# openMVG/openMVG

Measured on AMD Instinct MI355X. Metric: descriptor pairs/s (brute-force L2 2-NN + ratio matching), higher is better.
Workload: dtype i8 (int32 accumulate); 1 GPU; 1000 images x 2000 SIFT-like uint8x128 descriptors, exhaustive pairs (499500 image pairs, 499500 on rank 0), ratio 0.8; parallelism=pair-sharded x1, no collective

## Files before the change

### openmvg_amd/csrc/mvgx_bruteforce.hip

```cpp
#include <hip/hip_runtime.h>

#include <algorithm>
#include <cmath>
#include <cstring>
#include <deque>
#include <mutex>
#include <random>
#include <thread>
#include <vector>

#include "mvgx_buffers.h"
#include "mvgx_common.h"
#include "mvgx_match_batch.h"

namespace {

using mvgx::DevBuf;
using mvgx::PinnedBuf;
using mvgx::set_error;

constexpr int kQBlock = 256;
constexpr uint32_t kRowBits = 22;

struct HamParams {
// ... 546 lines not shown
      norms[r] = nn;
    }
    if ((rc = c->d_norms.ensure(norms.size()))) return rc;
    MVGX_HIP(hipMemcpyAsync(c->d_norms.p, norms.data(), norms.size() * sizeof(uint32_t), hipMemcpyHostToDevice, c->stream));
  }
  if (n_images)
    MVGX_HIP(hipMemcpyAsync(c->d_n.p, c->h_n.data(), n_images * sizeof(uint32_t), hipMemcpyHostToDevice, c->stream));
  MVGX_HIP(hipStreamSynchronize(c->stream));
  return MVGX_OK;
}

int bf_run(BfCtx* c, const uint32_t* pairs_IJ, uint64_t n_pairs, float ratio, mvgx_match_stats* stats) {
  MVGX_REQUIRE(c && (pairs_IJ || n_pairs == 0), MVGX_ERR_ARG, "run: NULL argument");
  MVGX_REQUIRE(c->nw != 0 || c->n_images == 0, MVGX_ERR_STATE, "run before set_regions");
  int rc;
  if (c->kind != 3 && (rc = check_ratio(ratio, "ratio"))) return rc;
  MVGX_HIP(hipSetDevice(c->device));
  if ((rc = check_pairs_in_range(pairs_IJ, n_pairs, c->n_images, "run"))) return rc;
  c->res_offsets.assign(n_pairs + 1, 0);
  c->res_ij.clear();
  mvgx_match_stats st;
  memset(&st, 0, sizeof(st));
  st.variant = (c->kind == 0 ? 100 : c->kind == 1 ? 200 : c->kind == 2 ? 300 : 400) + c->nw;
  float kernel_ms = 0.f;
  MVGX_HIP(hipEventRecord(c->ev0, c->stream));
  const uint64_t B = batch_size(c->batch_pairs, c->qstride);
  MVGX_REQUIRE(B * std::max<uint32_t>(c->qstride, 1) < (1ull << 32), MVGX_ERR_UNSUPPORTED,
               "images of %u descriptor slots: a 16-pair batch overflows the 32-bit match offsets of the device path", c->qstride);
  for (uint64_t p0 = 0; p0 < n_pairs; p0 += B) {
    const uint32_t nb = (uint32_t)std::min<uint64_t>(B, n_pairs - p0);
    const uint32_t blocks_per_pair = std::max<uint32_t>(1, c->qstride / kQBlock);
    if ((rc = c->hp_pairs.ensure(nb)) || (rc = c->hp_work.ensure((size_t)nb * blocks_per_pair))) return rc;
    uint32_t n_work = 0;
    for (uint32_t k = 0; k < nb; ++k) {
      const uint32_t I = pairs_IJ[2 * (p0 + k)], J = pairs_IJ[2 * (p0 + k) + 1];
      c->hp_pairs.p[k] = make_uint2(I, J);
      const uint32_t nI = c->h_n[I], nJ = c->h_n[J];
      if (c->kind == 3 ? (nI == 0 || nJ == 0) : (nI < 2 || nJ == 0)) continue;
      for (uint32_t q0 = 0; q0 < nJ; q0 += kQBlock) c->hp_work.p[n_work++] = make_uint2(k, q0);
      st.n_pairs += 1;
      st.n_desc_pairs += (uint64_t)nI * nJ;
    }
    if ((rc = c->d_pairs.ensure(nb)) || (rc = c->d_work.ensure(std::max<uint32_t>(n_work, 1))) ||
        (rc = c->d_best.ensure((size_t)nb * std::max<uint32_t>(c->qstride, 1))) || (rc = c->d_count.ensure(nb)) ||
        (rc = c->d_offsets.ensure((size_t)nb + 1)) || (rc = c->hp_offsets.ensure((size_t)nb + 1)))
      return rc;
    MVGX_HIP(hipMemcpyAsync(c->d_pairs.p, c->hp_pairs.p, nb * sizeof(uint2), hipMemcpyHostToDevice, c->stream));
    if (n_work) MVGX_HIP(hipMemcpyAsync(c->d_work.p, c->hp_work.p, n_work * sizeof(uint2), hipMemcpyHostToDevice, c->stream));
    MVGX_HIP(hipMemsetAsync(c->d_count.p, 0, nb * sizeof(uint32_t), c->stream));
    if (n_work) {
      MVGX_HIP(hipEventRecord(c->evk0, c->stream));
      if (c->kind == 3) {
        CasParams cp;
        cp.words = c->d_words.p; cp.hash = reinterpret_cast<const uint32_t*>(c->d_hash.p); cp.bids = c->d_bids.p; cp.bstart = c->d_bstart.p; cp.items = c->d_items.p;
        cp.img_row_off = c->d_row_off.p; cp.img_n = c->d_n.p; cp.pairs = c->d_pairs.p; cp.work = c->d_work.p; cp.best = c->d_best.p;
        cp.count = c->d_count.p; cp.qstride = c->qstride; cp.n_groups = c->cas_groups; cp.n_buckets = c->cas_buckets; cp.ratio_sq = ratio;
        if (c->cas_float) hipLaunchKernelGGL((cascade_match_kernel<64, 2, true>), dim3(n_work), dim3(kQBlock), 0, c->stream, cp);
        else if (c->nw == 36) hipLaunchKernelGGL((cascade_match_kernel<36, 5, false>), dim3(n_work), dim3(kQBlock), 0, c->stream, cp);
        else hipLaunchKernelGGL((cascade_match_kernel<32, 4, false>), dim3(n_work), dim3(kQBlock), 0, c->stream, cp);
      } else if (c->kind == 0) {
        HamParams hp;
        hp.words = c->d_words.p; hp.img_row_off = c->d_row_off.p; hp.img_n = c->d_n.p; hp.pairs = c->d_pairs.p; hp.work = c->d_work.p;
        hp.best = c->d_best.p; hp.count = c->d_count.p; hp.qstride = c->qstride; hp.ratio = ratio;
        if (c->nw == 8) hipLaunchKernelGGL(hamming_top2_ratio_kernel<8>, dim3(n_work), dim3(kQBlock), 0, c->stream, hp);
        else hipLaunchKernelGGL(hamming_top2_ratio_kernel<16>, dim3(n_work), dim3(kQBlock), 0, c->stream, hp);
      } else if (c->kind == 2) {
        L2uParams up;
        up.words = c->d_words.p; up.norms = c->d_norms.p; up.img_row_off = c->d_row_off.p; up.img_n = c->d_n.p; up.pairs = c->d_pairs.p;
        up.work = c->d_work.p; up.best = c->d_best.p; up.count = c->d_count.p; up.qstride = c->qstride; up.ratio_sq = ratio;
        if (c->nw == 16) hipLaunchKernelGGL(l2u8_top2_ratio_kernel<16>, dim3(n_work), dim3(kQBlock), 0, c->stream, up);
        else if (c->nw == 32) hipLaunchKernelGGL(l2u8_top2_ratio_kernel<32>, dim3(n_work), dim3(kQBlock), 0, c->stream, up);
        else hipLaunchKernelGGL(l2u8_top2_ratio_kernel<36>, dim3(n_work), dim3(kQBlock), 0, c->stream, up);
      } else {
        L2fParams fp;
        fp.rows = reinterpret_cast<const float*>(c->d_words.p); fp.img_row_off = c->d_row_off.p; fp.img_n = c->d_n.p;
        fp.pairs = c->d_pairs.p; fp.work = c->d_work.p; fp.best = c->d_best.p; fp.count = c->d_count.p; fp.qstride = c->qstride;
        fp.ratio_sq = ratio;
        hipLaunchKernelGGL(l2f_top2_ratio_kernel<64>, dim3(n_work), dim3(kQBlock), 0, c->stream, fp);
      }
      MVGX_HIP(hipGetLastError());
      MVGX_HIP(hipEventRecord(c->evk1, c->stream));
      st.n_kernel_launches += 1;
    }
    hipLaunchKernelGGL(scan_counts_kernel, dim3(1), dim3(1024), 0, c->stream, c->d_count.p, nb, c->d_offsets.p);
    MVGX_HIP(hipGetLastError());
    MVGX_HIP(hipMemcpyAsync(c->hp_offsets.p, c->d_offsets.p, ((size_t)nb + 1) * sizeof(uint32_t), hipMemcpyDeviceToHost, c->stream));
    MVGX_HIP(hipStreamSynchronize(c->stream));
    if (n_work) {
      float ms = 0.f;
      MVGX_HIP(hipEventElapsedTime(&ms, c->evk0, c->evk1));
      kernel_ms += ms;
    }
    const uint32_t total = c->hp_offsets.p[nb];
    const uint64_t base = c->res_offsets[p0];
    for (uint32_t k = 0; k <= nb; ++k) c->res_offsets[p0 + k] = base + c->hp_offsets.p[k];
    st.n_matches += total;
    if (total) {
      if ((rc = c->d_ij.ensure(total))) return rc;
      hipLaunchKernelGGL(compact_matches_kernel, dim3((nb + 3) / 4), dim3(256), 0, c->stream, c->d_best.p, c->d_offsets.p, c->d_pairs.p,
                         c->d_n.p, c->d_row_off.p, (const uint32_t*)nullptr, nb, c->qstride, c->d_ij.p);
      MVGX_HIP(hipGetLastError());
      const size_t old = c->res_ij.size();
      c->res_ij.resize(old + (size_t)total * 2);
      MVGX_HIP(hipMemcpyAsync(c->res_ij.data() + old, c->d_ij.p, (size_t)total * sizeof(uint2), hipMemcpyDeviceToHost, c->stream));
      MVGX_HIP(hipStreamSynchronize(c->stream));
    }
  }
  MVGX_HIP(hipEventRecord(c->ev1, c->stream));
  MVGX_HIP(hipEventSynchronize(c->ev1));
  float ms = 0.f;
  MVGX_HIP(hipEventElapsedTime(&ms, c->ev0, c->ev1));
  st.total_ms = ms;
  st.kernel_ms = kernel_ms;
  if (stats) *stats = st;
  return MVGX_OK;
}

template <typename Ctx>
int bf_create_as(int kind, int device, Ctx** out) {
  MVGX_REQUIRE(out, MVGX_ERR_ARG, "create: NULL out");
  *out = nullptr;
  Ctx* c = new Ctx();
  const int rc = bf_create(kind, device, c);
  if (rc) { delete c; return rc; }
  *out = c;
  return MVGX_OK;
}

}

extern "C" {

int mvgx_hamming_create(int device, mvgx_hamming_ctx** out) { return bf_create_as(0, device, out); }
int mvgx_hamming_destroy(mvgx_hamming_ctx* c) { delete c; return MVGX_OK; }
int mvgx_hamming_set_option(mvgx_hamming_ctx* c, const char* key, int64_t value) { return bf_set_option(c, key, value); }

int mvgx_hamming_set_regions(mvgx_hamming_ctx* c, const uint8_t* const* desc_rows, const uint32_t* n_desc, uint32_t n_images,
                             uint32_t desc_bytes) {
  MVGX_REQUIRE(c && (n_images == 0 || (desc_rows && n_desc)), MVGX_ERR_ARG, "mvgx_hamming_set_regions: NULL argument");
  MVGX_REQUIRE(desc_bytes >= 1 && desc_bytes <= 64, MVGX_ERR_UNSUPPORTED,
               "binary descriptor of %u bytes unsupported (device path: 1..64 bytes; AKAZE MLDB is 64)", desc_bytes);
  return bf_set_regions(c, desc_rows, n_desc, n_images, desc_bytes, desc_bytes <= 32 ? 8 : 16);
}

int mvgx_hamming_run(mvgx_hamming_ctx* c, const uint32_t* pairs_IJ, uint64_t n_pairs, float dist_ratio, mvgx_match_stats* stats) {
  return bf_run(c, pairs_IJ, n_pairs, dist_ratio, stats);
}

int mvgx_hamming_results(mvgx_hamming_ctx* c, const uint64_t** offsets, const uint32_t** ij) {
  MVGX_REQUIRE(c && offsets && ij, MVGX_ERR_ARG, "mvgx_hamming_results: NULL argument");
  *offsets = c->res_offsets.data();
  *ij = c->res_ij.data();
  return MVGX_OK;
}

int mvgx_l2f_create(int device, mvgx_l2f_ctx** out) { return bf_create_as(1, device, out); }
int mvgx_l2f_destroy(mvgx_l2f_ctx* c) { delete c; return MVGX_OK; }
int mvgx_l2f_set_option(mvgx_l2f_ctx* c, const char* key, int64_t value) { return bf_set_option(c, key, value); }

int mvgx_l2f_set_regions(mvgx_l2f_ctx* c, const float* const* desc_rows, const uint32_t* n_desc, uint32_t n_images, uint32_t dim) {
  MVGX_REQUIRE(c && (n_images == 0 || (desc_rows && n_desc)), MVGX_ERR_ARG, "mvgx_l2f_set_regions: NULL argument");
  MVGX_REQUIRE(dim == 64, MVGX_ERR_UNSUPPORTED,
               "float descriptors of length %u unsupported (device path: 64 = AKAZE_Float_Regions)", dim);
  return bf_set_regions(c, reinterpret_cast<const uint8_t* const*>(desc_rows), n_desc, n_images, dim * 4, dim);
}

int mvgx_l2f_run(mvgx_l2f_ctx* c, const uint32_t* pairs_IJ, uint64_t n_pairs, float ratio_sq, mvgx_match_stats* stats) {
// ... 243 lines not shown
```

### openmvg_amd/csrc/mvgx_match.hip

```cpp
#include <hip/hip_runtime.h>

#include <algorithm>
#include <atomic>
#include <climits>
#include <condition_variable>
#include <cstdint>
#include <cstdlib>
#include <cstring>
#include <functional>
#include <mutex>
#include <string>
#include <thread>
#include <vector>

#include "mvgx_buffers.h"
#include "mvgx_common.h"
#include "mvgx_match_batch.h"

namespace {

using mvgx::DevBuf;
using mvgx::PinnedBuf;
using mvgx::set_error;

// ... 895 lines not shown
    const int8_t* qsrc = p.tiles + (size_t)(tileJ0 + qt0) * kTileBytes + lane_chunk;
#pragma unroll
    for (int n = 0; n < kNBh; ++n)
#pragma unroll
      for (int ks = 0; ks < 2; ++ks) b[n][ks] = *reinterpret_cast<const v4i*>(qsrc + (n >> 1) * kTileBytes + (n & 1) * 256 + ks * 2048);
  }
  const int8_t* gI = p.tiles + (size_t)tileI0 * kTileBytes;
  const int* gC = p.cinit + (size_t)tileI0 * kTileRows;

  uint32_t qperm[kNBh];
  int qn[kNBh];
#pragma unroll
  for (int n = 0; n < kNBh; ++n) {
    const bool inb = lane < 16 && qt0 + (uint32_t)(n >> 1) < ntJpad;
    const size_t qs = (size_t)tileJ0 * kTileRows + (qt0 + (uint32_t)(n >> 1)) * kTileRows + (uint32_t)(n & 1) * 16 + (uint32_t)(lane & 15);
    qperm[n] = inb ? p.perm[qs] : kNoMatch;
    qn[n] = inb ? p.qnorm[qs] : 0;
  }

  int TP[kNBh][4], TW[kNBh][4], Q1[kNBh], Q2[kNBh], Qg[kNBh];
#pragma unroll
  for (int n = 0; n < kNBh; ++n) {
#pragma unroll
    for (int c = 0; c < 4; ++c) { TP[n][c] = kNegInit; TW[n][c] = kNegInit; }
    Q1[n] = kNegInit; Q2[n] = kNegInit; Qg[n] = 0;
  }

  stage_half_glds_asm(smem, gI, gC, wave, lane);
#pragma unroll
  for (int n = 0; n < kNBh; ++n) {
#pragma unroll
    for (int ks = 0; ks < 2; ++ks) asm volatile("" : "+v"(b[n][ks]));
    asm volatile("" : "+v"(qperm[n]), "+v"(qn[n]));
  }

  for (int hw = 0; hw < nhalf; ++hw) {
    asm volatile("s_waitcnt vmcnt(0)" ::: "memory");
    __syncthreads();
    char* buf = smem + (hw & 1) * kHalfStageBytes;
    char* nbuf = smem + ((hw + 1) & 1) * kHalfStageBytes;
    if (hw + 1 < nhalf)
      stage_half_glds_asm(nbuf, gI + (size_t)(hw + 1) * kHalfTiles * kTileBytes, gC + (hw + 1) * kHalfTiles * kTileRows, wave, lane);

    const int nt = min(kHalfTiles, ntI - hw * kHalfTiles);
    const char* wb = buf + lane_chunk;
    const char* wc = buf + kHalfTiles * kTileBytes + g4 * 16;
    v4i accA[4], accB[4];
#pragma unroll
    for (int i = 0; i < 4; ++i) accB[i] = v4i{kNegInit, kNegInit, kNegInit, kNegInit};
    v4i a0[2], a1[2], c0, c1;
    a0[0] = *reinterpret_cast<const v4i*>(wb);
    a0[1] = *reinterpret_cast<const v4i*>(wb + 2048);
    c0 = *reinterpret_cast<const v4i*>(wc);
    for (int t = 0; t < nt; ++t) {
      const int tn = min(t + 1, nt - 1);
      MVGX_GROUP16(accA, 0, a0, c0)
      a1[0] = *reinterpret_cast<const v4i*>(wb + t * kTileBytes + 256);
      a1[1] = *reinterpret_cast<const v4i*>(wb + t * kTileBytes + 256 + 2048);
      c1 = *reinterpret_cast<const v4i*>(wc + t * (kTileRows * 4) + 64);
      MVGX_EPI16(accB, 0, 1)
      MVGX_MIX16(3)
      MVGX_GROUP16(accB, 0, a1, c1)
      a0[0] = *reinterpret_cast<const v4i*>(wb + tn * kTileBytes);
      a0[1] = *reinterpret_cast<const v4i*>(wb + tn * kTileBytes + 2048);
      c0 = *reinterpret_cast<const v4i*>(wc + tn * (kTileRows * 4));
      MVGX_EPI16(accA, 0, 0)
      MVGX_MIX16(3)
    }
    MVGX_EPI16(accB, 0, 1)
    if ((hw & 1) || hw + 1 == nhalf) {
#pragma unroll
      for (int n = 0; n < kNBh; ++n) fold_window<4>(TW[n], TP[n], Q1[n], Q2[n], Qg[n], hw >> 1);
    }
  }

#pragma unroll
  for (int n = 0; n < kNBh; ++n) MVGX_FINISH16(n, qt0 + (uint32_t)(n >> 1) < ntJpad, qperm[n] != kNoMatch)
}
#undef MVGX_FINISH16
#undef MVGX_GROUP16
#undef MVGX_EPI16
#undef MVGX_MIX16

__device__ __forceinline__ int sum8_dpp(int v) {
  v += __builtin_amdgcn_update_dpp(0, v, 0xB1, 0xF, 0xF, true);
  v += __builtin_amdgcn_update_dpp(0, v, 0x4E, 0xF, 0xF, true);
  v += __builtin_amdgcn_update_dpp(0, v, 0x141, 0xF, 0xF, true);
  return v;
}
__device__ __forceinline__ int min16_dpp(int v) {
  v = min(v, __builtin_amdgcn_update_dpp(INT_MAX, v, 0xB1, 0xF, 0xF, false));
  v = min(v, __builtin_amdgcn_update_dpp(INT_MAX, v, 0x4E, 0xF, 0xF, false));
  v = min(v, __builtin_amdgcn_update_dpp(INT_MAX, v, 0x141, 0xF, 0xF, false));
  v = min(v, __builtin_amdgcn_update_dpp(INT_MAX, v, 0x140, 0xF, 0xF, false));
  return v;
}

template <bool kWaveUnits>
__global__ __launch_bounds__(256) void l2_verify_kernel(MatchParams p) {
  const int lane = threadIdx.x & 63;
  const int wave = threadIdx.x >> 6;
  uint32_t pair, qt0, I, tileI0, tileJ0, qend;
  const uint8_t* rowsJ = nullptr;
  if constexpr (kWaveUnits) {
    const uint4* rec = p.work8 + (size_t)kRecQuads * blockIdx.x;
    const uint4 wun = rec[1 + __builtin_amdgcn_readfirstlane(wave)];
    pair = wun.x; tileJ0 = wun.y; qt0 = wun.z; qend = wun.w;
    tileI0 = rec[0].x;
    const uint2 ij = p.pairs[pair];
    I = ij.x;
    rowsJ = p.rows_u8 + p.img_row_off[ij.y] * kDim;
  } else {
    const uint2 wk = p.work[blockIdx.x];
    const uint2 ij = p.pairs[wk.x];
    pair = wk.x; qt0 = wk.y + (uint32_t)wave * kNQ;
    I = ij.x;
    tileI0 = p.img_tile_off[I]; tileJ0 = p.img_tile_off[ij.y];
    qend = (p.img_tile_off[ij.y + 1] - tileJ0) * kTileRows;
  }
  const uint32_t nEvenI = p.img_neven[I], nOddI = p.img_n[I] - nEvenI;
  const int l16 = lane & 15, sub = lane >> 4;
  uint32_t accepted = 0;
  for (int part = 0; part < 2; ++part) {
    const uint32_t q0 = qt0 * kTileRows + (uint32_t)part * 64;
    const uint32_t q = q0 + lane;
    const bool inb = q < qend;
    const uint32_t code = inb ? p.best[(size_t)pair * p.qstride + q] : kNoMatch;
    unsigned long long todo = __ballot(code != kNoMatch);
    while (todo) {
      unsigned long long m = todo;
      for (int i = 0; i < sub; ++i) m &= m - 1;
      const bool active = m != 0;
      const int src = active ? __builtin_ctzll(m) : 0;
      for (int i = 0; i < 4; ++i) todo &= todo - 1;
      const uint32_t cc = (uint32_t)__shfl((int)code, src);
      const uint32_t qs = q0 + (uint32_t)src;
      const int s1 = cc & 7, hw = (cc >> 3) & 1, g1 = (int)(cc >> 4);
      const int piece = l16 & 7, rsel = l16 >> 3;
      const int mrow = slot_row(2 * s1 + rsel, hw);
      const size_t slot0 = (size_t)tileI0 * kTileRows + (active ? (size_t)g1 * kWinTiles * kTileRows + mrow : 0);
      const size_t slotQ = (size_t)tileJ0 * kTileRows + (active ? qs : 0);
      const size_t o = (size_t)pair * p.qstride + (active ? qs : 0);
      const uint32_t tt = (uint32_t)g1 * kWinTiles + (uint32_t)piece;
      const size_t slotI = active ? slot0 + (size_t)piece * kTileRows : slot0;
      const bool valid = active && (tt * 16u + (uint32_t)(2 * s1 + rsel)) < (hw ? nOddI : nEvenI);
      int4 va[8];
#pragma unroll
      for (int c = 0; c < 8; ++c)
        va[c] = *reinterpret_cast<const int4*>(p.rows_slot + (slot0 + (active ? (size_t)c * kTileRows : 0)) * kDim + piece * 16);
      int4 vb;
      if constexpr (kWaveUnits) {
        vb = *reinterpret_cast<const int4*>(rowsJ + (size_t)(active ? qs : 0) * kDim + piece * 16);
        vb.x ^= (int)0x80808080u; vb.y ^= (int)0x80808080u; vb.z ^= (int)0x80808080u; vb.w ^= (int)0x80808080u;
      } else {
        vb = *reinterpret_cast<const int4*>(p.rows_slot + slotQ * kDim + piece * 16);
      }
      const int2 f = p.cd[o];
      const int f_d0 = f.x, f_d1 = f.y;
      int nb = __builtin_amdgcn_sdot4(vb.x, vb.x, 0, false);
      nb = __builtin_amdgcn_sdot4(vb.y, vb.y, nb, false);
      nb = __builtin_amdgcn_sdot4(vb.z, vb.z, nb, false);
      nb = __builtin_amdgcn_sdot4(vb.w, vb.w, nb, false);
      nb = sum8_dpp(nb);
      int dot = 0, na = 0;
#pragma unroll
      for (int c = 0; c < 8; ++c) {
        int part = __builtin_amdgcn_sdot4(va[c].x, vb.x, 0, false);
        part = __builtin_amdgcn_sdot4(va[c].y, vb.y, part, false);
        part = __builtin_amdgcn_sdot4(va[c].z, vb.z, part, false);
        part = __builtin_amdgcn_sdot4(va[c].w, vb.w, part, false);
        part = sum8_dpp(part);
        dot = (c == piece) ? part : dot;
        int sq = __builtin_amdgcn_sdot4(va[c].x, va[c].x, 0, false);
        sq = __builtin_amdgcn_sdot4(va[c].y, va[c].y, sq, false);
        sq = __builtin_amdgcn_sdot4(va[c].z, va[c].z, sq, false);
        sq = __builtin_amdgcn_sdot4(va[c].w, va[c].w, sq, false);
        sq = sum8_dpp(sq);
        na = (c == piece) ? sq : na;
      }
      const int d = valid ? na + nb - 2 * dot : INT_MAX;
      const int key = min16_dpp(valid ? ((d << 4) | l16) : INT_MAX);
      const int wl = key & 15, dbest = key >> 4;
      const int second = min16_dpp((l16 == wl) ? INT_MAX : d);
      bool ok = false;
      if (active && l16 == wl) {
        if (key == INT_MAX || dbest != f_d0) atomicAdd(p.errflag, 1u);
        const int d1 = min(f_d1, second);
        ok = __int2float_rn(dbest) < __fmul_rn(p.ratio_sq, __int2float_rn(d1));
        p.best[o] = ok ? p.perm[slotI] : kNoMatch;
      }
      accepted += (uint32_t)__popcll(__ballot(ok));
    }
  }
  if (lane == 0 && accepted) atomicAdd(&p.count[pair], accepted);
}

__global__ __launch_bounds__(256) void count_candidates_kernel(const uint32_t* __restrict__ best, size_t n,
                                                               uint32_t* __restrict__ counter) {
  __shared__ uint32_t s_sum;
  if (threadIdx.x == 0) s_sum = 0;
  __syncthreads();
  uint32_t c = 0;
  const size_t base = (size_t)blockIdx.x * 16384;
  for (int k = 0; k < 64; ++k) {
    const size_t i = base + (size_t)k * 256 + threadIdx.x;
    if (i < n && best[i] != kNoMatch) ++c;
  }
  const unsigned long long m = __ballot(c != 0);
  (void)m;
  for (int off = 32; off > 0; off >>= 1) c += __shfl_down(c, off);
  if ((threadIdx.x & 63) == 0 && c) atomicAdd(&s_sum, c);
  __syncthreads();
  if (threadIdx.x == 0 && s_sum) atomicAdd(counter, s_sum);
}

__global__ __launch_bounds__(256) void count_candidates_units_kernel(MatchParams p, uint32_t* __restrict__ counter) {
  __shared__ uint32_t s_sum;
  if (threadIdx.x == 0) s_sum = 0;
  __syncthreads();
  const int lane = threadIdx.x & 63, wave = threadIdx.x >> 6;
  const uint4 wun = p.work8[(size_t)kRecQuads * blockIdx.x + 1 + wave];
  uint32_t c = 0;
  for (int part = 0; part < 2; ++part) {
    const uint32_t q = wun.z * kTileRows + (uint32_t)part * 64 + (uint32_t)lane;
    const bool cand = q < wun.w && p.best[(size_t)wun.x * p.qstride + q] != kNoMatch;
    c += (uint32_t)__popcll(__ballot(cand));
  }
  if (lane == 0 && c) atomicAdd(&s_sum, c);
  __syncthreads();
  if (threadIdx.x == 0 && s_sum) atomicAdd(counter, s_sum);
}

__global__ __launch_bounds__(256) void l2_top2_ratio_naive_kernel(MatchParams p) {
  const uint2 wk = p.work[blockIdx.x];
  const uint2 ij = p.pairs[wk.x];
  const uint32_t I = ij.x, J = ij.y;
  const uint32_t nI = p.img_n[I], nJ = p.img_n[J];
  const uint8_t* rowsI = p.rows_u8 + p.img_row_off[I] * kDim;
  const uint8_t* rowsJ = p.rows_u8 + p.img_row_off[J] * kDim;
  for (uint32_t q = wk.y * kTileRows + threadIdx.x; q < min(nJ, (wk.y + kBlockQTiles) * kTileRows);
       q += blockDim.x) {
    uint32_t qv[32];
#pragma unroll
    for (int k = 0; k < 32; ++k) qv[k] = reinterpret_cast<const uint32_t*>(rowsJ + (size_t)q * kDim)[k];
    int d0 = INT_MAX, d1 = INT_MAX;
    uint32_t i0 = 0;
    for (uint32_t i = 0; i < nI; ++i) {
      const uint32_t* dbr = reinterpret_cast<const uint32_t*>(rowsI + (size_t)i * kDim);
      int d = 0;
#pragma unroll
      for (int k = 0; k < 32; ++k) {
        const uint32_t x = qv[k], y = dbr[k];
#pragma unroll
        for (int bb = 0; bb < 4; ++bb) {
          const int df = (int)((x >> (8 * bb)) & 0xFF) - (int)((y >> (8 * bb)) & 0xFF);
          d += df * df;
        }
      }
      if (d < d0) { d1 = d0; d0 = d; i0 = i; }
      else if (d < d1) { d1 = d; }
    }
    const bool ok = __int2float_rn(d0) < __fmul_rn(p.ratio_sq, __int2float_rn(d1));
    p.best[(size_t)wk.x * p.qstride + p.rowpos[p.img_row_off[J] + q]] = ok ? i0 : kNoMatch;
    if (ok) atomicAdd(&p.count[wk.x], 1u);
  }
}


}

struct mvgx_match_ctx {
  int device = 0;
// ... 110 lines not shown
      out[2 * n] = make_uint4(k, qt, c->h_tile_off[I], c->h_tile_off[J]);
      out[2 * n + 1] = make_uint4(c->h_ntiles[I], c->h_tile_off[J + 1] - c->h_tile_off[J], 0, 0);
      ++n;
    }
  }
  return n;
}
uint32_t build_records(const mvgx_match_ctx* c, const uint32_t* ij, uint32_t nb, uint4* out) {
  uint32_t n_rec = 0, rec_used = kWaves, rec_I = 0;
  for (uint32_t k = 0; k < nb; ++k) {
    const uint32_t I = ij[2 * k], J = ij[2 * k + 1];
    if (!pair_has_work(c, I, J)) continue;
    const uint32_t ntJq = c->h_qtile_off[J + 1] - c->h_qtile_off[J];
    for (uint32_t qt = 0; qt < ntJq; qt += kNQ) {
      if (rec_used == kWaves || rec_I != I) {
        uint4* r = out + (size_t)kRecQuads * n_rec++;
        r[0] = make_uint4(c->h_tile_off[I], c->h_ntiles[I], 0, 0);
        for (int w = 0; w < kWaves; ++w) r[1 + w] = make_uint4(0, c->h_qtile_off[I], 0, 0);
        rec_used = 0; rec_I = I;
      }
      out[(size_t)kRecQuads * (n_rec - 1) + 1 + rec_used++] = make_uint4(k, c->h_qtile_off[J], qt, c->h_n[J]);
    }
  }
  return n_rec;
}

template <typename T>
int upload_list(DevBuf<T>& d, const PinnedBuf<T>& h, size_t n, hipStream_t stream) {
  const int rc = d.ensure(std::max<size_t>(n, 1));
  if (rc) return rc;
  if (n) MVGX_HIP(hipMemcpyAsync(d.p, h.p, n * sizeof(T), hipMemcpyHostToDevice, stream));
  return MVGX_OK;
}

int prep_regions(mvgx_match_ctx* c) {
  const uint32_t n_images = c->n_images;
  c->h_tile_off.assign(n_images + 1, 0);
  c->h_row_off.assign(n_images + 1, 0);
  c->h_ntiles.assign(n_images + 1, 0);
  c->h_qtile_off.assign(n_images + 1, 0);
  uint32_t max_n = 0;
  for (uint32_t k = 0; k < n_images; ++k) {
    c->h_row_off[k + 1] = c->h_row_off[k] + c->h_n[k];
    c->h_qtile_off[k + 1] = c->h_qtile_off[k] + (c->h_n[k] + kTileRows - 1) / kTileRows;
    max_n = std::max(max_n, c->h_n[k]);
  }
  const uint64_t total_rows = c->h_row_off[n_images];
  int rc;
  if ((rc = c->d_row_off.ensure(n_images + 1))) return rc;
  if ((rc = c->d_tile_off.ensure(n_images + 1))) return rc;
  if ((rc = c->d_qtile_off.ensure(n_images + 1))) return rc;
  if ((rc = c->d_n.ensure(n_images + 1))) return rc;
  if ((rc = c->d_ntiles.ensure(n_images + 1))) return rc;
  if ((rc = c->d_neven.ensure(n_images + 1))) return rc;
  if ((rc = c->d_err.ensure(2))) return rc;
  if ((rc = c->d_rownorm.ensure(std::max<uint64_t>(total_rows, 1)))) return rc;
  if ((rc = c->d_rowpos.ensure(std::max<uint64_t>(total_rows, 1)))) return rc;
  MVGX_HIP(hipMemcpyAsync(c->d_row_off.p, c->h_row_off.data(), (n_images + 1) * sizeof(uint64_t),
                          hipMemcpyHostToDevice, c->stream));
  MVGX_HIP(hipMemcpyAsync(c->d_n.p, c->h_n.data(), n_images * sizeof(uint32_t), hipMemcpyHostToDevice, c->stream));
  MVGX_HIP(hipMemsetAsync(c->d_neven.p, 0, (n_images + 1) * sizeof(uint32_t), c->stream));
  MVGX_HIP(hipMemsetAsync(c->d_err.p, 0, 2 * sizeof(uint32_t), c->stream));
  std::vector<uint32_t> h_even(n_images + 1, 0);
  if (total_rows > 0) {
    dim3 grid((max_n + 255) / 256, n_images);
    hipLaunchKernelGGL(row_norms_kernel, grid, dim3(256), 0, c->stream, c->d_rows_view, c->d_row_off.p, c->d_n.p,
                       c->d_rownorm.p, c->d_neven.p);
    MVGX_HIP(hipGetLastError());
    MVGX_HIP(hipMemcpyAsync(h_even.data(), c->d_neven.p, n_images * sizeof(uint32_t), hipMemcpyDeviceToHost, c->stream));
  }
  MVGX_HIP(hipStreamSynchronize(c->stream));
  uint32_t max_pad = 0;
  for (uint32_t k = 0; k < n_images; ++k) {
    const uint32_t ne = h_even[k], no = c->h_n[k] - h_even[k];
    const uint32_t nt = (std::max(ne, no) + 15) / 16;
    const uint32_t pad = (nt + kWinTiles - 1) / kWinTiles * kWinTiles;
    c->h_ntiles[k] = nt;
    c->h_tile_off[k + 1] = c->h_tile_off[k] + pad;
    max_pad = std::max(max_pad, pad);
  }
  c->total_tiles = c->h_tile_off[n_images];
  c->max_tiles_pad = max_pad;
  c->qstride = max_pad * kTileRows;
  const size_t alloc_tiles = (size_t)c->total_tiles + kTailTiles;
  const size_t alloc_slots = alloc_tiles * kTileRows;
  if ((rc = c->d_tiles.ensure(alloc_tiles * kTileBytes))) return rc;
  if ((rc = c->d_rows_slot.ensure(alloc_tiles * kTileBytes))) return rc;
  if ((rc = c->d_rconst.ensure(alloc_slots))) return rc;
  if ((rc = c->d_cinit.ensure(alloc_slots))) return rc;
  if ((rc = c->d_qnorm.ensure(alloc_slots))) return rc;
  if ((rc = c->d_perm.ensure(alloc_slots))) return rc;
  const size_t total_qtiles = c->h_qtile_off[n_images];
  if ((rc = c->d_qtiles.ensure((total_qtiles + kTailTiles) * kTileBytes))) return rc;
  if ((rc = c->d_qtnorm.ensure((total_qtiles + kTailTiles) * kTileRows))) return rc;
  MVGX_HIP(hipMemcpyAsync(c->d_qtile_off.p, c->h_qtile_off.data(), (n_images + 1) * sizeof(uint32_t), hipMemcpyHostToDevice, c->stream));
  MVGX_HIP(hipMemsetAsync(c->d_qtiles.p + total_qtiles * kTileBytes, 0, (size_t)kTailTiles * kTileBytes, c->stream));
  MVGX_HIP(hipMemsetAsync(c->d_qtnorm.p + total_qtiles * kTileRows, 0, (size_t)kTailTiles * kTileRows * sizeof(int), c->stream));
  MVGX_HIP(hipMemcpyAsync(c->d_tile_off.p, c->h_tile_off.data(), (n_images + 1) * sizeof(uint32_t),
                          hipMemcpyHostToDevice, c->stream));
  MVGX_HIP(hipMemcpyAsync(c->d_ntiles.p, c->h_ntiles.data(), (n_images + 1) * sizeof(uint32_t),
                          hipMemcpyHostToDevice, c->stream));
  const int fill_grid = (int)((alloc_slots + 255) / 256);
  hipLaunchKernelGGL(fill_i32_kernel, dim3(fill_grid), dim3(256), 0, c->stream, c->d_rconst.p, alloc_slots, kRPad);
  hipLaunchKernelGGL(fill_i32_kernel, dim3(fill_grid), dim3(256), 0, c->stream, c->d_cinit.p, alloc_slots, kCPad);
  hipLaunchKernelGGL(fill_i32_kernel, dim3(fill_grid), dim3(256), 0, c->stream, c->d_qnorm.p, alloc_slots, 0);
  hipLaunchKernelGGL(fill_i32_kernel, dim3(fill_grid), dim3(256), 0, c->stream, reinterpret_cast<int*>(c->d_perm.p),
                     alloc_slots, (int)kNoMatch);
  MVGX_HIP(hipGetLastError());
  MVGX_HIP(hipMemsetAsync(c->d_tiles.p + (size_t)c->total_tiles * kTileBytes, 0, (size_t)kTailTiles * kTileBytes,
                          c->stream));
  if (total_rows > 0 && max_pad > 0) {
    hipLaunchKernelGGL(assign_slots_kernel, dim3(n_images), dim3(1024), 0, c->stream, c->d_row_off.p, c->d_tile_off.p,
                       c->d_n.p, c->d_rownorm.p, c->d_rowpos.p, c->d_perm.p, c->d_rconst.p, c->d_cinit.p, c->d_qnorm.p);
    MVGX_HIP(hipGetLastError());
    dim3 grid(max_pad, n_images);
    hipLaunchKernelGGL(build_tiles_kernel, grid, dim3(256), 0, c->stream, c->d_rows_view, c->d_row_off.p,
                       c->d_tile_off.p, c->d_perm.p, c->d_tiles.p, c->d_rows_slot.p);
    MVGX_HIP(hipGetLastError());
    dim3 qgrid((max_n + kTileRows - 1) / kTileRows, n_images);
    hipLaunchKernelGGL(build_qtiles_kernel, qgrid, dim3(256), 0, c->stream, c->d_rows_view, c->d_row_off.p, c->d_qtile_off.p, c->d_n.p,
                       c->d_rownorm.p, c->d_qtiles.p, c->d_qtnorm.p);
    MVGX_HIP(hipGetLastError());
  }
  MVGX_HIP(hipStreamSynchronize(c->stream));
  return MVGX_OK;
}

hipEvent_t get_event(mvgx_match_ctx* c, size_t i) {
  while (c->ev_pool.size() <= i) {
    hipEvent_t e = nullptr;
    if (hipEventCreate(&e) != hipSuccess) return nullptr;
    c->ev_pool.push_back(e);
  }
  return c->ev_pool[i];
}

}

extern "C" {

int mvgx_match_create_multi(const int* devices, int n_devices, mvgx_match_ctx** out) {
  MVGX_REQUIRE(out != nullptr && devices != nullptr && n_devices >= 1, MVGX_ERR_ARG, "mvgx_match_create_multi: bad argument");
  if (n_devices == 1) return mvgx_match_create(devices[0] < 0 ? -2 : devices[0], out);
  auto* c = new mvgx_match_ctx();
  c->device = devices[0];
  for (int k = 0; k < n_devices; ++k) {
    mvgx_match_ctx* child = nullptr;
    const int rc = mvgx_match_create(devices[k] < 0 ? -2 : devices[k], &child);
    if (rc) { mvgx_match_destroy(c); return rc; }
    c->children.push_back(child);
  }
  *out = c;
  return MVGX_OK;
}

int mvgx_match_create(int device, mvgx_match_ctx** out) {
  MVGX_REQUIRE(out != nullptr, MVGX_ERR_ARG, "mvgx_match_create: out is NULL");
  if (device == -1) {
    std::vector<int> devs;
    int rc = mvgx::devices_from_env(devs);
    if (rc) return rc;
    if (devs.size() >= 2) return mvgx_match_create_multi(devs.data(), (int)devs.size(), out);
    if (devs.size() == 1) device = devs[0];
  }
  if (device < 0) device = -1;
  int rc = mvgx::select_device(device);
// ... 204 lines not shown
  int rc;

  MVGX_HIP(hipEventRecord(c->ev_total0, c->slot[0].stream));

  const KernelForm form = resolve_form(c);
  auto issue = [&](mvgx_match_ctx::Slot& sl, mvgx_match_ctx::Slot* prev, uint64_t p0, uint32_t nb) -> int {
    int rc;
    hipStream_t stream = sl.stream;
    sl.p0 = p0; sl.nb = nb;
    const uint32_t* ij = pairs_IJ + 2 * p0;
    if ((rc = sl.hp_pairs.ensure(nb))) return rc;
    for (uint32_t k = 0; k < nb; ++k) {
      const uint32_t I = ij[2 * k], J = ij[2 * k + 1];
      sl.hp_pairs.p[k] = make_uint2(I, J);
      if (!pair_has_work(c, I, J)) continue;
      st.n_pairs += 1;
      st.n_desc_pairs += (uint64_t)c->h_n[I] * c->h_n[J];
    }
    const size_t max_items16 = (size_t)nb * std::max<uint32_t>(1, (c->max_tiles_pad + kBlockQTiles - 1) / kBlockQTiles);
    uint32_t n_list[3] = {0, 0, 0};
    if (form.reads(kListItems16)) {
      if ((rc = sl.hp_work.ensure(max_items16))) return rc;
      n_list[kListItems16] = build_items16(c, ij, nb, sl.hp_work.p);
    }
    if (form.reads(kListItems8h)) {
      if ((rc = sl.hp_work8h.ensure(max_items16 * 4))) return rc;
      n_list[kListItems8h] = build_items8h(c, ij, nb, sl.hp_work8h.p);
    }
    if (form.reads(kListRecords)) {
      if ((rc = sl.hp_work8.ensure(max_items16 * kRecQuads))) return rc;
      n_list[kListRecords] = build_records(c, ij, nb, sl.hp_work8.p);
    }
    const uint32_t n_filter = n_list[form.list], n_verify = n_list[form.verify_list];
    if ((rc = sl.d_pairs.ensure(nb))) return rc;
    if ((rc = sl.d_best.ensure((size_t)nb * c->qstride))) return rc;
    if (form.verify && (rc = sl.d_cd.ensure((size_t)nb * c->qstride))) return rc;
    if ((rc = sl.d_count.ensure(nb))) return rc;
    if ((rc = sl.d_offsets.ensure((size_t)nb + 1))) return rc;
    if ((rc = sl.hp_offsets.ensure((size_t)nb + 1))) return rc;
    MVGX_HIP(hipMemcpyAsync(sl.d_pairs.p, sl.hp_pairs.p, nb * sizeof(uint2), hipMemcpyHostToDevice, stream));
    if (form.reads(kListItems16) && (rc = upload_list(sl.d_work, sl.hp_work, n_list[kListItems16], stream))) return rc;
    if (form.reads(kListItems8h) && (rc = upload_list(sl.d_work8h, sl.hp_work8h, (size_t)n_list[kListItems8h] * 2, stream))) return rc;
    if (form.reads(kListRecords) && (rc = upload_list(sl.d_work8, sl.hp_work8, (size_t)n_list[kListRecords] * kRecQuads, stream))) return rc;
    MVGX_HIP(hipMemsetAsync(sl.d_count.p, 0, nb * sizeof(uint32_t), stream));

    MatchParams mp;
    mp.tiles = c->d_tiles.p; mp.rows_slot = c->d_rows_slot.p; mp.rconst = c->d_rconst.p; mp.cinit = c->d_cinit.p; mp.qnorm = c->d_qnorm.p;
    mp.perm = c->d_perm.p; mp.rowpos = c->d_rowpos.p; mp.qtiles = c->d_qtiles.p; mp.qtnorm = c->d_qtnorm.p;
    mp.rows_u8 = c->d_rows_view; mp.img_row_off = c->d_row_off.p;
    mp.img_tile_off = c->d_tile_off.p; mp.img_n = c->d_n.p; mp.img_ntiles = c->d_ntiles.p;
    mp.cd = sl.d_cd.p; mp.img_neven = c->d_neven.p; mp.errflag = c->d_err.p;
    mp.pairs = sl.d_pairs.p; mp.work = sl.d_work.p; mp.work8 = sl.d_work8.p; mp.work8h = sl.d_work8h.p; mp.n_work = n_filter;
    mp.best = sl.d_best.p; mp.count = sl.d_count.p; mp.qstride = c->qstride; mp.ratio_sq = ratio_sq;

    if (prev) MVGX_HIP(hipStreamWaitEvent(stream, prev->ev_filter, 0));
    if (n_filter) {
      hipEvent_t e0 = nullptr, e1 = nullptr;
      if (c->profile) {
        e0 = get_event(c, n_ev++); e1 = get_event(c, n_ev++);
        MVGX_REQUIRE(e0 && e1, MVGX_ERR_HIP, "hipEventCreate failed");
        MVGX_HIP(hipEventRecord(e0, stream));
      }
      hipLaunchKernelGGL(form.filter, dim3(n_filter), dim3(256), form.lds_bytes, stream, mp);
      MVGX_HIP(hipGetLastError());
      if (c->profile) MVGX_HIP(hipEventRecord(e1, stream));
      if (!c->verify_alone) MVGX_HIP(hipEventRecord(sl.ev_filter, stream));
      st.n_kernel_launches += 1;
      if (form.verify) {
        if (c->profile >= 2) {
          const size_t nslots = (size_t)nb * c->qstride;
          if (form.count_units)
            hipLaunchKernelGGL(count_candidates_units_kernel, dim3(n_verify), dim3(256), 0, stream, mp, c->d_err.p + 1);
          else
            hipLaunchKernelGGL(count_candidates_kernel, dim3((unsigned)((nslots + 16383) / 16384)), dim3(256), 0, stream,
                               mp.best, nslots, c->d_err.p + 1);
        }
        hipLaunchKernelGGL(form.verify, dim3(n_verify), dim3(256), 0, stream, mp);
        MVGX_HIP(hipGetLastError());
      }
      if (c->verify_alone) MVGX_HIP(hipEventRecord(sl.ev_filter, stream));
    }
    if (!n_filter) MVGX_HIP(hipEventRecord(sl.ev_filter, stream));
    uint32_t* const d_offsets = sl.d_offsets.p;
    hipLaunchKernelGGL(scan_counts_kernel, dim3(1), dim3(1024), 0, stream, mp.count, nb, d_offsets);
    MVGX_HIP(hipGetLastError());
    MVGX_HIP(hipMemcpyAsync(sl.hp_offsets.p, sl.d_offsets.p, ((size_t)nb + 1) * sizeof(uint32_t), hipMemcpyDeviceToHost, stream));
    MVGX_HIP(hipEventRecord(sl.ev_scan, stream));
    return MVGX_OK;
  };
  auto finish = [&](mvgx_match_ctx::Slot& sl) -> int {
    int rc;
    MVGX_HIP(hipEventSynchronize(sl.ev_scan));
    const uint32_t nb = sl.nb;
    const uint64_t p0 = sl.p0;
    const uint32_t total = sl.hp_offsets.p[nb];
    if (sink) {
      if (c->stream_hold) sl.out_set ^= 1;
      sl.h_off_out[sl.out_set].assign(sl.hp_offsets.p, sl.hp_offsets.p + nb + 1);
    } else {
      const uint64_t base = res.offsets[p0];
      for (uint32_t k = 0; k <= nb; ++k) res.offsets[p0 + k] = base + sl.hp_offsets.p[k];
    }
    sl.out_p0 = p0; sl.out_nb = nb;
    st.n_matches += total;
    if (total) {
      if ((rc = sl.d_ij.ensure(total))) return rc;
      hipStream_t stream = sl.stream;
      const uint32_t *d_best = sl.d_best.p, *d_offsets = sl.d_offsets.p;
      const uint2* d_pairs = sl.d_pairs.p;
      uint2* d_ij = sl.d_ij.p;
      hipLaunchKernelGGL(compact_matches_kernel, dim3((nb + 3) / 4), dim3(256), 0, stream, d_best, d_offsets, d_pairs, c->d_n.p,
                         c->d_row_off.p, form.dense_slots ? nullptr : c->d_rowpos.p, nb, c->qstride, d_ij);
      MVGX_HIP(hipGetLastError());
      if (sink) {
        PinnedBuf<uint32_t>& hb = sl.hp_ij[sl.out_set];
        if (!hb.p) hb.pageable = !c->pinned_stream;
        if ((size_t)total * 2 > hb.cap) { hb.release(); if ((rc = hb.grow_keep(std::max<size_t>((size_t)total * 3, 4u << 20), 0))) return rc; }
        MVGX_HIP(hipMemcpyAsync(hb.p, sl.d_ij.p, (size_t)total * sizeof(uint2), hipMemcpyDeviceToHost, sl.stream));
      } else if (c->keep_host_results) {
        const size_t old = res.ij_n;
        if (old + (size_t)total * 2 > res.ij.cap)
          for (auto& o : c->slot) MVGX_HIP(hipStreamSynchronize(o.stream));
        if ((rc = res.ij.grow_keep(old + (size_t)total * 2, old))) return rc;
        res.ij_n = old + (size_t)total * 2;
        MVGX_HIP(hipMemcpyAsync(res.ij.p + old, sl.d_ij.p, (size_t)total * sizeof(uint2),
                                hipMemcpyDeviceToHost, sl.stream));
      }
    }
    if (sink) MVGX_HIP(hipEventRecord(sl.ev_copy, sl.stream));
    return MVGX_OK;
  };
  auto deliver = [&](mvgx_match_ctx::Slot& sl) -> int {
    MVGX_HIP(hipEventSynchronize(sl.ev_copy));
    if (feed.stop.load()) return MVGX_OK;
    if ((*sink)(sl.out_p0, sl.out_nb, sl.h_off_out[sl.out_set].data(), sl.hp_ij[sl.out_set].p)) feed.stop.store(1);
    return MVGX_OK;
  };
  uint64_t nbatch = 0, p0 = 0;
  uint32_t nb = 0;
  while (feed.take(p0, nb)) {
    mvgx_match_ctx::Slot& cur = c->slot[nbatch & 1];
    mvgx_match_ctx::Slot* prev = nbatch ? &c->slot[(nbatch - 1) & 1] : nullptr;
    if (!c->overlap) {
      if ((rc = issue(cur, nullptr, p0, nb)) || (rc = finish(cur))) return rc;
      MVGX_HIP(hipStreamSynchronize(cur.stream));
      if (sink && (rc = deliver(cur))) return rc;
      ++nbatch;
      continue;
    }
    if ((rc = issue(cur, prev, p0, nb))) return rc;
    if (prev && (rc = finish(*prev))) return rc;
    if (sink && nbatch >= 2 && (rc = deliver(cur))) return rc;
    ++nbatch;
  }
  if (c->overlap && nbatch) {
    mvgx_match_ctx::Slot& last = c->slot[(nbatch - 1) & 1];
    if (sink && nbatch >= 2 && (rc = deliver(c->slot[nbatch & 1]))) return rc;
    if ((rc = finish(last))) return rc;
    if (sink && (rc = deliver(last))) return rc;
  }
  for (auto& sl : c->slot) MVGX_HIP(hipStreamSynchronize(sl.stream));
  MVGX_HIP(hipEventRecord(c->ev_total1, c->slot[0].stream));
  MVGX_HIP(hipEventSynchronize(c->ev_total1));
  float ms = 0.f;
  MVGX_HIP(hipEventElapsedTime(&ms, c->ev_total0, c->ev_total1));
  st.total_ms = ms;
  if (form.verify) {
    uint32_t flags[2] = {0, 0};
    MVGX_HIP(hipMemcpy(flags, c->d_err.p, 2 * sizeof(uint32_t), hipMemcpyDeviceToHost));
// ... 182 lines not shown
```

### openmvg_amd/csrc/mvgx_match_batch.h

```cpp
#pragma once
#include <hip/hip_runtime.h>

#include <algorithm>
#include <cstdint>

#include "mvgx_common.h"

namespace {

constexpr uint32_t kNoMatch = 0xFFFFFFFFu;

__global__ __launch_bounds__(1024) void scan_counts_kernel(const uint32_t* __restrict__ count, uint32_t n,
                                                           uint32_t* __restrict__ offsets ) {
  __shared__ uint32_t s_part[1024];
  const uint32_t per = (n + 1023) / 1024;
  const uint32_t lo = min(n, threadIdx.x * per), hi = min(n, lo + per);
  uint32_t sum = 0;
  for (uint32_t i = lo; i < hi; ++i) sum += count[i];
  s_part[threadIdx.x] = sum;
  __syncthreads();
  for (uint32_t d = 1; d < 1024; d <<= 1) {
    const uint32_t v = (threadIdx.x >= d) ? s_part[threadIdx.x - d] : 0;
    __syncthreads();
    s_part[threadIdx.x] += v;
    __syncthreads();
  }
  uint32_t run = s_part[threadIdx.x] - sum;
  for (uint32_t i = lo; i < hi; ++i) { offsets[i] = run; run += count[i]; }
  if (threadIdx.x == 1023) offsets[n] = s_part[1023];
}

__global__ __launch_bounds__(256) void compact_matches_kernel(const uint32_t* __restrict__ best,
                                                              const uint32_t* __restrict__ offsets,
                                                              const uint2* __restrict__ pairs,
                                                              const uint32_t* __restrict__ img_n,
                                                              const uint64_t* __restrict__ img_row_off,
                                                              const uint32_t* __restrict__ rowpos,
                                                              uint32_t n_pairs, uint32_t qstride,
                                                              uint2* __restrict__ out_ij) {
  const uint32_t pidx = blockIdx.x * 4 + (threadIdx.x >> 6);
  if (pidx >= n_pairs) return;
  const int lane = threadIdx.x & 63;
  const uint32_t off = offsets[pidx];
  if (offsets[pidx + 1] == off) return;
  const uint32_t J = pairs[pidx].y;
  const uint32_t nJ = img_n[J];
  const uint32_t* pos = rowpos ? rowpos + img_row_off[J] : nullptr;
  uint32_t run = off;
  for (uint32_t q0 = 0; q0 < nJ; q0 += 64) {
    const uint32_t q = q0 + lane;
    const uint32_t v = (q < nJ) ? best[(size_t)pidx * qstride + (pos ? pos[q] : q)] : kNoMatch;
    const bool ok = v != kNoMatch;
    const unsigned long long m = __ballot(ok);
    if (ok) {
      const uint32_t pre = (uint32_t)__popcll(m & ((1ull << lane) - 1ull));
      out_ij[run + pre] = make_uint2(v, q);
    }
    run += (uint32_t)__popcll(m);
  }
}

inline uint64_t batch_size(int64_t batch_pairs, uint32_t qstride) {
  return std::max<uint64_t>(1, std::min<uint64_t>((uint64_t)batch_pairs, std::max<uint64_t>(16, (1ull << 29) / std::max<uint32_t>(qstride, 1))));
}

inline int check_pairs_in_range(const uint32_t* pairs_IJ, uint64_t n_pairs, uint32_t n_images, const char* who) {
  for (uint64_t k = 0; k < n_pairs; ++k)
    MVGX_REQUIRE(pairs_IJ[2 * k] < n_images && pairs_IJ[2 * k + 1] < n_images, MVGX_ERR_ARG,
                 "%s: pair %llu references image out of range", who, (unsigned long long)k);
  return MVGX_OK;
}

inline int check_ratio(float ratio, const char* who) {
  MVGX_REQUIRE(ratio <= 1.0f && ratio >= 0.0f, MVGX_ERR_UNSUPPORTED,
               "%s = %g: the device path reproduces the reference only for 0 <= %s <= 1 "
               "(ties are libstdc++ partial_sort order beyond that)", who, (double)ratio, who);
  return MVGX_OK;
}

}
```

Measured before the change: 10520 billion descriptor pairs/s.

## Compact verify candidates via LDS, use precomputed norms, and write scan offsets to host directly

The L2 verify kernel now compacts candidate queries into a per-wave shared-memory list instead of iterating a ballot mask. It reads precomputed query norms (qtnorm/qnorm) and row norms (cinit) instead of recomputing squared norms with sdot4, and replaces eight per-chunk DPP reductions with a butterfly transpose-reduce. The scan kernel also writes offsets straight into pinned host memory, removing a separate device-to-host memcpy. This saves ALU and DPP work plus one copy, at the cost of LDS use, wave-level fences, uncached host writes from the GPU, and a new limit on tile count.

```diff
diff --git a/openmvg_amd/csrc/mvgx_bruteforce.hip b/openmvg_amd/csrc/mvgx_bruteforce.hip
--- a/openmvg_amd/csrc/mvgx_bruteforce.hip
+++ b/openmvg_amd/csrc/mvgx_bruteforce.hip
@@ -652,7 +652,7 @@
       MVGX_HIP(hipEventRecord(c->evk1, c->stream));
       st.n_kernel_launches += 1;
     }
-    hipLaunchKernelGGL(scan_counts_kernel, dim3(1), dim3(1024), 0, c->stream, c->d_count.p, nb, c->d_offsets.p);
+    hipLaunchKernelGGL(scan_counts_kernel, dim3(1), dim3(1024), 0, c->stream, c->d_count.p, nb, c->d_offsets.p, (uint32_t*)nullptr);
     MVGX_HIP(hipGetLastError());
     MVGX_HIP(hipMemcpyAsync(c->hp_offsets.p, c->d_offsets.p, ((size_t)nb + 1) * sizeof(uint32_t), hipMemcpyDeviceToHost, c->stream));
     MVGX_HIP(hipStreamSynchronize(c->stream));
diff --git a/openmvg_amd/csrc/mvgx_match.hip b/openmvg_amd/csrc/mvgx_match.hip
--- a/openmvg_amd/csrc/mvgx_match.hip
+++ b/openmvg_amd/csrc/mvgx_match.hip
@@ -1001,12 +1001,6 @@
 #undef MVGX_EPI16
 #undef MVGX_MIX16
 
-__device__ __forceinline__ int sum8_dpp(int v) {
-  v += __builtin_amdgcn_update_dpp(0, v, 0xB1, 0xF, 0xF, true);
-  v += __builtin_amdgcn_update_dpp(0, v, 0x4E, 0xF, 0xF, true);
-  v += __builtin_amdgcn_update_dpp(0, v, 0x141, 0xF, 0xF, true);
-  return v;
-}
 __device__ __forceinline__ int min16_dpp(int v) {
   v = min(v, __builtin_amdgcn_update_dpp(INT_MAX, v, 0xB1, 0xF, 0xF, false));
   v = min(v, __builtin_amdgcn_update_dpp(INT_MAX, v, 0x4E, 0xF, 0xF, false));
@@ -1037,66 +1031,80 @@
     tileI0 = p.img_tile_off[I]; tileJ0 = p.img_tile_off[ij.y];
     qend = (p.img_tile_off[ij.y + 1] - tileJ0) * kTileRows;
   }
+  __shared__ uint2 s_pend[kWaves][64];
   const uint32_t nEvenI = p.img_neven[I], nOddI = p.img_n[I] - nEvenI;
   const int l16 = lane & 15, sub = lane >> 4;
+  const int piece = l16 & 7, rsel = l16 >> 3;
+  const int8_t* rowsI = p.rows_slot + (size_t)tileI0 * kTileBytes;
+  const int* cinitI = p.cinit + (size_t)tileI0 * kTileRows;
+  const uint32_t* permI = p.perm + (size_t)tileI0 * kTileRows;
   uint32_t accepted = 0;
   for (int part = 0; part < 2; ++part) {
     const uint32_t q0 = qt0 * kTileRows + (uint32_t)part * 64;
     const uint32_t q = q0 + lane;
     const bool inb = q < qend;
     const uint32_t code = inb ? p.best[(size_t)pair * p.qstride + q] : kNoMatch;
-    unsigned long long todo = __ballot(code != kNoMatch);
-    while (todo) {
-      unsigned long long m = todo;
-      for (int i = 0; i < sub; ++i) m &= m - 1;
-      const bool active = m != 0;
-      const int src = active ? __builtin_ctzll(m) : 0;
-      for (int i = 0; i < 4; ++i) todo &= todo - 1;
-      const uint32_t cc = (uint32_t)__shfl((int)code, src);
-      const uint32_t qs = q0 + (uint32_t)src;
-      const int s1 = cc & 7, hw = (cc >> 3) & 1, g1 = (int)(cc >> 4);
-      const int piece = l16 & 7, rsel = l16 >> 3;
+    const bool cand = code != kNoMatch;
+    const unsigned long long pend = __ballot(cand);
+    const int n_pend = __popcll(pend);
+    __builtin_amdgcn_fence(__ATOMIC_RELEASE, "wavefront");
+    __builtin_amdgcn_wave_barrier();
+    if (cand) s_pend[wave][__popcll(pend & ((1ull << lane) - 1ull))] = make_uint2(code, (uint32_t)lane);
+    __builtin_amdgcn_fence(__ATOMIC_RELEASE, "wavefront");
+    __builtin_amdgcn_wave_barrier();
+    __builtin_amdgcn_fence(__ATOMIC_ACQUIRE, "wavefront");
+    for (int k0 = 0; k0 < n_pend; k0 += 4) {
+      const bool active = k0 + sub < n_pend;
+      const uint2 pc = s_pend[wave][active ? k0 + sub : k0];
+      const uint32_t cc = pc.x;
+      const uint32_t qs = q0 + pc.y;
+      const int s1 = cc & 7, hw = (cc >> 3) & 1;
+      const uint32_t g1 = cc >> 4;
       const int mrow = slot_row(2 * s1 + rsel, hw);
-      const size_t slot0 = (size_t)tileI0 * kTileRows + (active ? (size_t)g1 * kWinTiles * kTileRows + mrow : 0);
-      const size_t slotQ = (size_t)tileJ0 * kTileRows + (active ? qs : 0);
-      const size_t o = (size_t)pair * p.qstride + (active ? qs : 0);
-      const uint32_t tt = (uint32_t)g1 * kWinTiles + (uint32_t)piece;
-      const size_t slotI = active ? slot0 + (size_t)piece * kTileRows : slot0;
-      const bool valid = active && (tt * 16u + (uint32_t)(2 * s1 + rsel)) < (hw ? nOddI : nEvenI);
+      const uint32_t cell = g1 * (kWinTiles * kTileRows) + (uint32_t)mrow;
+      const uint32_t slotI = cell + (uint32_t)piece * kTileRows;
+      const uint32_t off0 = cell * kDim + (uint32_t)piece * 16;
+      const size_t slotQ = (size_t)tileJ0 * kTileRows + qs;
+      const size_t o = (size_t)pair * p.qstride + qs;
+      const uint32_t tt = g1 * kWinTiles + (uint32_t)piece;
+      const bool valid = (tt * 16u + (uint32_t)(2 * s1 + rsel)) < (hw ? nOddI : nEvenI);
       int4 va[8];
 #pragma unroll
       for (int c = 0; c < 8; ++c)
-        va[c] = *reinterpret_cast<const int4*>(p.rows_slot + (slot0 + (active ? (size_t)c * kTileRows : 0)) * kDim + piece * 16);
+        va[c] = *reinterpret_cast<const int4*>(rowsI + (off0 + (uint32_t)(c * kTileRows * kDim)));
       int4 vb;
+      int nb;
       if constexpr (kWaveUnits) {
-        vb = *reinterpret_cast<const int4*>(rowsJ + (size_t)(active ? qs : 0) * kDim + piece * 16);
+        vb = *reinterpret_cast<const int4*>(rowsJ + (size_t)qs * kDim + piece * 16);
         vb.x ^= (int)0x80808080u; vb.y ^= (int)0x80808080u; vb.z ^= (int)0x80808080u; vb.w ^= (int)0x80808080u;
+        nb = p.qtnorm[slotQ];
       } else {
         vb = *reinterpret_cast<const int4*>(p.rows_slot + slotQ * kDim + piece * 16);
+        nb = p.qnorm[slotQ];
       }
+      const int na = -2 * cinitI[slotI] + hw;
       const int2 f = p.cd[o];
       const int f_d0 = f.x, f_d1 = f.y;
-      int nb = __builtin_amdgcn_sdot4(vb.x, vb.x, 0, false);
-      nb = __builtin_amdgcn_sdot4(vb.y, vb.y, nb, false);
-      nb = __builtin_amdgcn_sdot4(vb.z, vb.z, nb, false);
-      nb = __builtin_amdgcn_sdot4(vb.w, vb.w, nb, false);
-      nb = sum8_dpp(nb);
-      int dot = 0, na = 0;
+      int pd[8];
 #pragma unroll
       for (int c = 0; c < 8; ++c) {
-        int part = __builtin_amdgcn_sdot4(va[c].x, vb.x, 0, false);
-        part = __builtin_amdgcn_sdot4(va[c].y, vb.y, part, false);
-        part = __builtin_amdgcn_sdot4(va[c].z, vb.z, part, false);
-        part = __builtin_amdgcn_sdot4(va[c].w, vb.w, part, false);
-        part = sum8_dpp(part);
-        dot = (c == piece) ? part : dot;
-        int sq = __builtin_amdgcn_sdot4(va[c].x, va[c].x, 0, false);
-        sq = __builtin_amdgcn_sdot4(va[c].y, va[c].y, sq, false);
-        sq = __builtin_amdgcn_sdot4(va[c].z, va[c].z, sq, false);
-        sq = __builtin_amdgcn_sdot4(va[c].w, va[c].w, sq, false);
-        sq = sum8_dpp(sq);
-        na = (c == piece) ? sq : na;
+        pd[c] = __builtin_amdgcn_sdot4(va[c].x, vb.x, 0, false);
+        pd[c] = __builtin_amdgcn_sdot4(va[c].y, vb.y, pd[c], false);
+        pd[c] = __builtin_amdgcn_sdot4(va[c].z, vb.z, pd[c], false);
+        pd[c] = __builtin_amdgcn_sdot4(va[c].w, vb.w, pd[c], false);
       }
+      const bool up4 = (piece & 4) != 0, up2 = (piece & 2) != 0, up1 = (piece & 1) != 0;
+#pragma unroll
+      for (int j = 0; j < 4; ++j) {
+        const int keep = up4 ? pd[4 + j] : pd[j], send = up4 ? pd[j] : pd[4 + j];
+        pd[j] = keep + __builtin_amdgcn_update_dpp(0, send, 0x141, 0xF, 0xF, true);
+      }
+#pragma unroll
+      for (int j = 0; j < 2; ++j) {
+        const int keep = up2 ? pd[2 + j] : pd[j], send = up2 ? pd[j] : pd[2 + j];
+        pd[j] = keep + __builtin_amdgcn_update_dpp(0, send, 0x4E, 0xF, 0xF, true);
+      }
+      const int dot = (up1 ? pd[1] : pd[0]) + __builtin_amdgcn_update_dpp(0, up1 ? pd[0] : pd[1], 0xB1, 0xF, 0xF, true);
       const int d = valid ? na + nb - 2 * dot : INT_MAX;
       const int key = min16_dpp(valid ? ((d << 4) | l16) : INT_MAX);
       const int wl = key & 15, dbest = key >> 4;
@@ -1106,7 +1114,7 @@
         if (key == INT_MAX || dbest != f_d0) atomicAdd(p.errflag, 1u);
         const int d1 = min(f_d1, second);
         ok = __int2float_rn(dbest) < __fmul_rn(p.ratio_sq, __int2float_rn(d1));
-        p.best[o] = ok ? p.perm[slotI] : kNoMatch;
+        p.best[o] = ok ? permI[slotI] : kNoMatch;
       }
       accepted += (uint32_t)__popcll(__ballot(ok));
     }
@@ -1383,6 +1391,7 @@
   c->total_tiles = c->h_tile_off[n_images];
   c->max_tiles_pad = max_pad;
   c->qstride = max_pad * kTileRows;
+  MVGX_REQUIRE(max_pad <= (1u << 20), MVGX_ERR_UNSUPPORTED, "an image of more than 2^24 descriptors of one norm parity is not supported");
   const size_t alloc_tiles = (size_t)c->total_tiles + kTailTiles;
   const size_t alloc_slots = alloc_tiles * kTileRows;
   if ((rc = c->d_tiles.ensure(alloc_tiles * kTileBytes))) return rc;
@@ -1753,9 +1762,9 @@
     }
     if (!n_filter) MVGX_HIP(hipEventRecord(sl.ev_filter, stream));
     uint32_t* const d_offsets = sl.d_offsets.p;
-    hipLaunchKernelGGL(scan_counts_kernel, dim3(1), dim3(1024), 0, stream, mp.count, nb, d_offsets);
+    uint32_t* const hp_offsets = sl.hp_offsets.p;
+    hipLaunchKernelGGL(scan_counts_kernel, dim3(1), dim3(1024), 0, stream, mp.count, nb, d_offsets, hp_offsets);
     MVGX_HIP(hipGetLastError());
-    MVGX_HIP(hipMemcpyAsync(sl.hp_offsets.p, sl.d_offsets.p, ((size_t)nb + 1) * sizeof(uint32_t), hipMemcpyDeviceToHost, stream));
     MVGX_HIP(hipEventRecord(sl.ev_scan, stream));
     return MVGX_OK;
   };
diff --git a/openmvg_amd/csrc/mvgx_match_batch.h b/openmvg_amd/csrc/mvgx_match_batch.h
--- a/openmvg_amd/csrc/mvgx_match_batch.h
+++ b/openmvg_amd/csrc/mvgx_match_batch.h
@@ -11,7 +11,8 @@
 constexpr uint32_t kNoMatch = 0xFFFFFFFFu;
 
 __global__ __launch_bounds__(1024) void scan_counts_kernel(const uint32_t* __restrict__ count, uint32_t n,
-                                                           uint32_t* __restrict__ offsets ) {
+                                                           uint32_t* __restrict__ offsets ,
+                                                           uint32_t* __restrict__ host_offsets ) {
   __shared__ uint32_t s_part[1024];
   const uint32_t per = (n + 1023) / 1024;
   const uint32_t lo = min(n, threadIdx.x * per), hi = min(n, lo + per);
@@ -26,8 +27,15 @@
     __syncthreads();
   }
   uint32_t run = s_part[threadIdx.x] - sum;
-  for (uint32_t i = lo; i < hi; ++i) { offsets[i] = run; run += count[i]; }
-  if (threadIdx.x == 1023) offsets[n] = s_part[1023];
+  for (uint32_t i = lo; i < hi; ++i) {
+    offsets[i] = run;
+    if (host_offsets) host_offsets[i] = run;
+    run += count[i];
+  }
+  if (threadIdx.x == 1023) {
+    offsets[n] = s_part[1023];
+    if (host_offsets) host_offsets[n] = s_part[1023];
+  }
 }
 
 __global__ __launch_bounds__(256) void compact_matches_kernel(const uint32_t* __restrict__ best,
```

After: 10560 billion descriptor pairs/s (median of 6 runs). Within noise of the previous version (+0.4%).
